# gabrielfnayres/new-vit

Measured on AMD Instinct MI355X. Metric: volumes_per_sec_mst_dinov2_fwd, higher is better.
Workload: dtype bf16; 1 GPU; MST-DINOv2 (DinoV2ClassifierSlice, ViT-S/14) forward, 4 volumes/GPU of 64x512x512 bf16 zero-padded to 518x518 (N=1370 tokens/slice); global_batch_volumes=4, slices=64, parallelism=single GPU, weights=synthetic (mst.synth seed 2), random init of the reference architecture

## Files before the change

### new-vit_amd/csrc/k_block16s.hip

```cpp
#include <type_traits>

#include "mst_common.h"

namespace {

constexpr int E = 384, HID = 1536, CH = 32;
constexpr int NCHUNK = HID / CH;
constexpr int PJ = E / CH;
constexpr int ELEM_BYTES = 24 * 1024;
constexpr int ELEMS = PJ + 2 * NCHUNK;
constexpr int NSLOT = 6;
constexpr int AHEAD = 4;
constexpr int RING_BYTES = NSLOT * ELEM_BYTES;
constexpr int B1_OFF = RING_BYTES;
constexpr int BP_OFF = B1_OFF + HID * 4;
constexpr int B2_OFF = BP_OFF + E * 4;
constexpr int LDS_BYTES = B2_OFF + E * 4;
constexpr int NF = 24;
#ifndef BLOCKS_DEPTH
#define BLOCKS_DEPTH 4
#endif
constexpr int D = BLOCKS_DEPTH;
constexpr int R = D + 2;
static_assert(NF % R == 0, "fragment ring must tile the phase");
#ifdef BLOCKS_PAIRS
constexpr int frag_of(int i) { return i; }
#else
constexpr int frag_of(int i) { return 2 * (i % 12) + i / 12; }
#endif
constexpr int BIAS_SLOT = 8;

template <int OFF, typename V> __device__ __forceinline__ void lds_read_b128(V& dst, unsigned addr) {
#if defined(BLOCKS_WACC)
    asm volatile("ds_read_b128 %0, %1 offset:%2" : "=a"(dst) : "v"(addr), "i"(OFF));
#elif !defined(BLOCKS_NOREADS)
    asm volatile("ds_read_b128 %0, %1 offset:%2" : "=v"(dst) : "v"(addr), "i"(OFF));
#else
    asm volatile("" : "=v"(dst) : "v"(addr));
#endif
}
template <int OFF, typename V> __device__ __forceinline__ void lds_read_b128_acc(V& dst, unsigned addr) {
    asm volatile("ds_read_b128 %0, %1 offset:%2" : "=a"(dst) : "v"(addr), "i"(OFF));
}
template <int N> __device__ __forceinline__ void wait_lgkm() {
    asm volatile("s_waitcnt lgkmcnt(%0)" ::"n"(N));
    __builtin_amdgcn_sched_barrier(0);
}
#ifdef BLOCKS_STAMPS
__device__ unsigned long long g_bsstamps[256 * 4 * 16];
__device__ __forceinline__ unsigned long long bstamp() {
    unsigned long long t;
    __builtin_amdgcn_sched_barrier(0);
    asm volatile("s_memtime %0\n\ts_waitcnt lgkmcnt(0)" : "=s"(t)::"memory");
    __builtin_amdgcn_sched_barrier(0);
    return t;
}
#define BST(var) const unsigned long long var = bstamp()
#define BACC(slot, a, b) st[slot] += (b) - (a)
#else
#define BST(var)
#define BACC(slot, a, b)
#endif

template <int I, int N, typename F> __device__ __forceinline__ void static_for(F&& f) {
    if constexpr (I < N) {
        f(std::integral_constant<int, I>{});
        static_for<I + 1, N>(f);
    }
}

__device__ __forceinline__ f32x16 cat16(f32x4 a, f32x4 b, f32x4 c, f32x4 d) {
    typedef __attribute__((ext_vector_type(8))) float f32x8;
    const f32x8 lo = __builtin_shufflevector(a, b, 0, 1, 2, 3, 4, 5, 6, 7), hi = __builtin_shufflevector(c, d, 0, 1, 2, 3, 4, 5, 6, 7);
    return __builtin_shufflevector(lo, hi, 0, 1, 2, 3, 4, 5, 6, 7, 8, 9, 10, 11, 12, 13, 14, 15);
}
template <int Q> __device__ __forceinline__ f32x4 sub4(f32x16 v) { return __builtin_shufflevector(v, v, 4 * Q, 4 * Q + 1, 4 * Q + 2, 4 * Q + 3); }

template <typename T> struct Gelu;
template <> struct Gelu<bf16_t> {
    static constexpr int STAGES = 7;
    static constexpr int target(int) { return 0; }
    template <int S> static __device__ __forceinline__ void stage(float v, float& a, float& b, float& c) {
        if constexpr (S == 0) a = v * v;
        else if constexpr (S == 1) a = fmaf(a, -0.06940179f * 1.4426950408889634f, -1.60031416f * 1.4426950408889634f);
        else if constexpr (S == 2) a = v * a;
        else if constexpr (S == 3) a = __builtin_amdgcn_exp2f(a);
        else if constexpr (S == 4) a = 1.0f + a;
        else if constexpr (S == 5) a = __builtin_amdgcn_rcpf(a);
        else a = v * a;
    }
};
template <> struct Gelu<f16_t> {
    static constexpr int STAGES = 9;
    static constexpr int target(int S) { return S == 0 ? 1 : (S == 2 || S == 3) ? 2 : 0; }
    template <int S> static __device__ __forceinline__ void stage(float v, float& a, float& b, float& c) {
        if constexpr (S == 0) b = __builtin_amdgcn_fmed3f(v, -8.0f, 8.0f);
        else if constexpr (S == 1) a = b * b;
        else if constexpr (S == 2) c = fmaf(a, 7.03033577e-04f * 1.4426950408889634f, -7.40112920e-02f * 1.4426950408889634f);
        else if constexpr (S == 3) c = fmaf(c, a, -1.59501577f * 1.4426950408889634f);
        else if constexpr (S == 4) a = b * c;
        else if constexpr (S == 5) a = __builtin_amdgcn_exp2f(a);
        else if constexpr (S == 6) a = 1.0f + a;
        else if constexpr (S == 7) a = __builtin_amdgcn_rcpf(a);
        else a = v * a;
    }
};

template <typename T>
__global__ __launch_bounds__(256) void block16s_kernel(float* x, const T* attn, T* xn_out, const char* __restrict__ wseq,
                                                       const float* __restrict__ b1f, const float* __restrict__ bproj,
                                                       const float* __restrict__ b2, int M, int ntiles, float eps, int layout) {
    typedef typename V8<T>::type vec8;
    typedef typename V8<T>::half_type vec4;
    extern __shared__ __attribute__((aligned(16))) char smem[];
    const bool x_in_img = layout & MST_LAYOUT_X_IN_IMAGE, x_out_img = layout & MST_LAYOUT_X_OUT_IMAGE, act_blk = layout & MST_LAYOUT_ACT_BLOCKED;
    const int tid = threadIdx.x, lane = tid & 63;
    const int wave = __builtin_amdgcn_readfirstlane(tid >> 6);
    const int row32 = lane & 31, half = lane >> 5;
    const unsigned lds_base = (unsigned)(uintptr_t)(__attribute__((address_space(3))) char*)smem;
    const unsigned lane16 = lane * 16;

    const int my_tiles = (ntiles - (int)blockIdx.x + (int)gridDim.x - 1) / (int)gridDim.x;
    if (my_tiles <= 0) return;

    for (int i = tid; i < HID / 4; i += 256) *reinterpret_cast<f32x4*>(smem + B1_OFF + i * 16) = *reinterpret_cast<const f32x4*>(b1f + 4 * i);
    for (int i = tid; i < E / 4; i += 256) {
        *reinterpret_cast<f32x4*>(smem + BP_OFF + i * 16) = *reinterpret_cast<const f32x4*>(bproj + 4 * i);
        *reinterpret_cast<f32x4*>(smem + B2_OFF + i * 16) = *reinterpret_cast<const f32x4*>(b2 + 4 * i);
    }
    asm volatile("s_waitcnt vmcnt(0) lgkmcnt(0)" ::: "memory");

#ifndef BLOCKS_DMA_GLOBAL
    const __amdgpu_buffer_rsrc_t wrsrc = __builtin_amdgcn_make_buffer_rsrc((void*)wseq, 0, ELEMS * ELEM_BYTES, 0x00020000);
    const int wlane_off = wave * 6144 + lane16;
    char* const wdst_wave = smem + wave * 6144;
    auto dma_piece = [&](int src_off, int slot, auto u_tag) {
        constexpr int u = decltype(u_tag)::value;
#ifndef BLOCKS_NODMA
        constexpr int hi = u >= 4 ? 4096 : 0;
        __builtin_amdgcn_raw_ptr_buffer_load_lds(wrsrc, LDS_PTR(wdst_wave + slot * ELEM_BYTES + hi), 16, wlane_off, src_off + hi, u * 1024 - hi, 0);
#endif
    };
#else
    const char* const wsrc_lane = wseq + (wave * 6144 + 2048) + lane16;
    char* const wdst_wave = smem + wave * 6144 + 2048;
    auto dma_piece = [&](int src_off, int slot, auto u_tag) {
        constexpr int u = decltype(u_tag)::value;
#ifndef BLOCKS_NODMA
        __builtin_amdgcn_global_load_lds(GLB_PTR(wsrc_lane + src_off), LDS_PTR(wdst_wave + slot * ELEM_BYTES), 16, (u - 2) * 1024, 0);
#endif
    };
#endif
    for (int e0 = 0; e0 < AHEAD; ++e0) static_for<0, 6>([&](auto u) { dma_piece(e0 * ELEM_BYTES, e0, u); });
    int dsrc = AHEAD * ELEM_BYTES, dslot = AHEAD;

    f32x16 acc[12];
    u32x4 xa[24];
    f32x4 hq[2][4];
    vec8 hB[2][2];
    vec8 w[R];
    float ga[8], gb[8], gc[8];
#ifdef BLOCKS_NOFILL
    hB[0][0] = hB[0][1] = hB[1][0] = hB[1][1] = vec8{};
#endif

    int slot = 0;
    const unsigned b1_lane = lds_base + B1_OFF + half * 16;

#ifdef BLOCKS_STAMPS
    unsigned long long st[16] = {0, 0, 0, 0, 0, 0, 0, 0, 0, 0, 0, 0, 0, 0, 0, 0};
    const unsigned long long tstart = bstamp();
#endif
    auto phase = [&](auto head_tag, auto tail_tag, auto bq_tag, int bias_chunk, auto&& mf, auto&& fill, auto cat_tag, auto ord_tag, auto nord_tag) {
        constexpr bool HEAD = decltype(head_tag)::value, TAIL = decltype(tail_tag)::value;
        constexpr int ORD = decltype(ord_tag)::value, NORD = decltype(nord_tag)::value;
        auto fr = [](int i, int ord) constexpr { return ord ? frag_of(i) : i; };
        constexpr int BQ = decltype(bq_tag)::value, CAT = decltype(cat_tag)::value;
        BST(p0);
        asm volatile("s_waitcnt vmcnt(12)\n\ts_barrier" ::: "memory");
        BST(p1);
        BACC(CAT, p0, p1);
        const unsigned cur = lds_base + slot * ELEM_BYTES + lane16;
        const int nslot = slot + 1 == NSLOT ? 0 : slot + 1;
        const unsigned nxt = lds_base + nslot * ELEM_BYTES + lane16;
        const int my_dsrc = dsrc, my_dslot = dslot;
        dsrc = dsrc + ELEM_BYTES == ELEMS * ELEM_BYTES ? 0 : dsrc + ELEM_BYTES;
        dslot = dslot + 1 == NSLOT ? 0 : dslot + 1;
        const unsigned baddr = b1_lane + 128 * bias_chunk;
        f32x4 bt0, bt1, bt2, bt3;
        if constexpr (HEAD) static_for<0, D>([&](auto q) { lds_read_b128<fr(decltype(q)::value, ORD) * 1024>(w[decltype(q)::value % R], cur); });
        static_for<0, NF>([&](auto it) {
            constexpr int i = decltype(it)::value;
            if constexpr (i + D < NF) lds_read_b128<fr(i + D, ORD) * 1024>(w[(i + D) % R], cur);
            else if constexpr (TAIL) lds_read_b128<fr(i + D - NF, NORD) * 1024>(w[(i + D) % R], nxt);
            if constexpr (BQ >= 0 && i == BIAS_SLOT) {
                lds_read_b128_acc<0>(bt0, baddr);
                lds_read_b128_acc<32>(bt1, baddr);
                lds_read_b128_acc<64>(bt2, baddr);
                lds_read_b128_acc<96>(bt3, baddr);
            }
#ifndef BLOCKS_WAIT1
            if constexpr (i % 2 == 0) {
                constexpr int last = TAIL ? i + D : (i + D < NF - 1 ? i + D : NF - 1);
                constexpr int younger_frags = last - (i + 1) > 0 ? last - (i + 1) : 0;
                constexpr int younger_bias = (BQ >= 0 && i >= BIAS_SLOT && i + 1 <= BIAS_SLOT + D) ? 4 : 0;
                wait_lgkm<younger_frags + younger_bias>();
            } else {
                __builtin_amdgcn_sched_barrier(0);
            }
#else
            constexpr int younger_frags = TAIL ? D : (NF - 1 - i < D ? NF - 1 - i : D);
            constexpr int younger_bias = (BQ >= 0 && i >= BIAS_SLOT && i <= BIAS_SLOT + D) ? 4 : 0;
            wait_lgkm<younger_frags + younger_bias>();
#endif
            if constexpr (BQ >= 0 && i == BIAS_SLOT + D + 1) {
                asm volatile("" : "+a"(bt0), "+a"(bt1), "+a"(bt2), "+a"(bt3));
                hq[BQ < 0 ? 0 : BQ][0] = bt0;
                hq[BQ < 0 ? 0 : BQ][1] = bt1;
                hq[BQ < 0 ? 0 : BQ][2] = bt2;
                hq[BQ < 0 ? 0 : BQ][3] = bt3;
            }
            mf(it, w[i % R]);
#ifdef BLOCKS_DMA_FRONT
            if constexpr (i == 0) static_for<0, 6>([&](auto u) { dma_piece(my_dsrc, my_dslot, u); });
#else
            if constexpr (i % 4 == 3) dma_piece(my_dsrc, my_dslot, std::integral_constant<int, i / 4>{});
#endif
            fill(it);
        });
        slot = nslot;
        BST(p2);
        BACC(CAT + 1, p1, p2);
    };
    constexpr std::integral_constant<int, 0> C_PROJ{};
    constexpr std::integral_constant<int, 2> C_A{};
    constexpr std::integral_constant<int, 4> C_B{};
    constexpr std::integral_constant<int, 6> C_G10{};
    auto no_fill = [](auto) {};
    constexpr std::true_type YES{};
    constexpr std::false_type NO{};
    constexpr std::integral_constant<int, -1> NOBIAS{};
    constexpr std::integral_constant<int, 0> I0{};
    constexpr std::integral_constant<int, 1> I1{};

    auto gemm1_mf = [&](auto hs_tag) {
        return [&](auto it, const vec8& wf) {
            constexpr int hs = decltype(hs_tag)::value, i = decltype(it)::value;
            f32x16 c = cat16(hq[hs][0], hq[hs][1], hq[hs][2], hq[hs][3]);
            c = mfma32(wf, __builtin_bit_cast(vec8, xa[i]), c);
            static_for<0, 4>([&](auto q) { hq[hs][decltype(q)::value] = sub4<decltype(q)::value>(c); });
        };
    };
    auto gemm2_mf = [&](auto hs_tag) {
        return [&](auto it, const vec8& wf) {
            constexpr int hs = decltype(hs_tag)::value, i = frag_of(decltype(it)::value);
            acc[i >> 1] = mfma32(wf, hB[hs][i & 1], acc[i >> 1]);
        };
    };

    constexpr int GOPS = 8 * Gelu<T>::STAGES + 4;
    auto gelu_op = [&](auto hs_tag, auto part_tag, auto n_tag) {
        constexpr int hs = decltype(hs_tag)::value, PART = decltype(part_tag)::value, n = decltype(n_tag)::value;
        if constexpr (n < 8 * Gelu<T>::STAGES) {
            constexpr int grp = n / (4 * Gelu<T>::STAGES), m = n % (4 * Gelu<T>::STAGES);
            constexpr int st = m / 4, val = 4 * grp + m % 4;
            Gelu<T>::template stage<st>(hq[hs][2 * PART + (val >> 2)][val & 3], ga[val], gb[val], gc[val]);
            if constexpr (Gelu<T>::target(st) == 0) asm volatile("" : "+v"(ga[val]));
            else if constexpr (Gelu<T>::target(st) == 1) asm volatile("" : "+v"(gb[val]));
            else asm volatile("" : "+v"(gc[val]));
        } else if constexpr (n < GOPS) {
            constexpr int pr = n - 8 * Gelu<T>::STAGES;
            hB[hs][PART][2 * pr] = (T)ga[2 * pr];
            hB[hs][PART][2 * pr + 1] = (T)ga[2 * pr + 1];
        }
    };
    constexpr int OPS_PER_SLOT = (GOPS + NF - 2) / (NF - 1);
    auto gelu_fill = [&](auto hs_tag, auto part_tag) {
        return [&, hs_tag, part_tag](auto it) {
            constexpr int i = decltype(it)::value;
#ifdef BLOCKS_NOFILL
            if constexpr (i == 12) static_for<0, 8>([&](auto e) { hB[decltype(hs_tag)::value][decltype(part_tag)::value][decltype(e)::value] = (T)hq[decltype(hs_tag)::value][2 * decltype(part_tag)::value + (decltype(e)::value >> 2)][decltype(e)::value & 3]; });
            if constexpr (false)
#else
            if constexpr (i >= 1)
#endif
                static_for<0, OPS_PER_SLOT>([&](auto o) { gelu_op(hs_tag, part_tag, std::integral_constant<int, (i - 1) * OPS_PER_SLOT + decltype(o)::value>{}); });
        };
    };
    auto gelu_now = [&](auto hs_tag, auto part_tag) { static_for<0, GOPS>([&](auto n) { gelu_op(hs_tag, part_tag, n); }); };

    const int last_grp = (M - 1) >> 5;
    auto row_of = [&](int tile) { const int g = tile * 128 + wave * 32 + row32; return (unsigned)(g < M ? g : M - 1); };
    auto grp_of = [&](int tile) { return (size_t)((tile * 4 + wave) < last_grp ? (tile * 4 + wave) : last_grp); };
    auto load_attn = [&](int tile) {
        if (act_blk) {
            const char* ap = (const char*)attn + (grp_of(tile) * (32 * E * 2) + lane16);
#pragma unroll
            for (int i = 0; i < 24; ++i) xa[i] = *reinterpret_cast<const u32x4*>(ap + 1024 * i);
        } else {
            const char* ap = (const char*)attn + ((size_t)row_of(tile) * (E * 2) + half * 16);
#pragma unroll
            for (int i = 0; i < 24; ++i) xa[i] = *reinterpret_cast<const u32x4*>(ap + 32 * i);
        }
    };
    auto load_x = [&](int tile, auto t_tag) {
        constexpr int t = decltype(t_tag)::value;
        const char* xp = x_in_img ? (const char*)x + (grp_of(tile) * (32 * E * 4) + lane16) + 4096 * t
                                  : (const char*)x + ((size_t)row_of(tile) * (E * 4) + half * 16) + 128 * t;
        const int qstep = x_in_img ? 1024 : 32;
#pragma unroll
        for (int q = 0; q < 4; ++q) {
            const f32x4 v = *reinterpret_cast<const f32x4*>(xp + qstep * q);
#pragma unroll
            for (int r = 0; r < 4; ++r) acc[t][4 * q + r] = v[r];
        }
    };
#ifndef BLOCKS_TILE_CYCLES
#define BLOCKS_TILE_CYCLES 170000
#endif
#ifndef BLOCKS_NO_DEPHASE
    if (my_tiles >= 4) {
        const int min_tiles = ntiles / (int)gridDim.x;
        const unsigned u = (((unsigned)blockIdx.x >> 3) + 5u * ((unsigned)blockIdx.x & 7u)) & 15u;
        const unsigned long long delay = (unsigned long long)BLOCKS_TILE_CYCLES * ((my_tiles > min_tiles ? 0u : 16u) + u) / 32u;
        const unsigned long long t0 = __builtin_readcyclecounter();
        for (int it = 0; it < 640 && __builtin_readcyclecounter() - t0 < delay; ++it) __builtin_amdgcn_s_sleep(32);
    }
#endif
    load_attn(blockIdx.x);
    static_for<0, 12>([&](auto t) { load_x(blockIdx.x, t); });

    for (int k = 0; k < my_tiles; ++k) {
        const int tile = blockIdx.x + k * gridDim.x;
        const int next_tile = k + 1 < my_tiles ? tile + (int)gridDim.x : tile;
        const int grow = tile * 128 + wave * 32 + row32;
        const bool valid = grow < M;
        const unsigned crow = (unsigned)(valid ? grow : M - 1);
        BST(q0);
        BST(q1);
        BACC(8, q0, q1);
        static_for<0, PJ>([&](auto jt) {
            constexpr int j = decltype(jt)::value;
            auto mf = [&](auto it, const vec8& wf) {
                constexpr int i = frag_of(decltype(it)::value);
                acc[i >> 1] = mfma32(wf, __builtin_bit_cast(vec8, xa[2 * j + (i & 1)]), acc[i >> 1]);
            };
            if constexpr (j == 0) phase(YES, YES, NOBIAS, 0, mf, no_fill, C_PROJ, I1, I1);
            else if constexpr (j == PJ - 1) phase(NO, NO, I0, 0, mf, no_fill, C_PROJ, I1, I1);
            else phase(NO, YES, NOBIAS, 0, mf, no_fill, C_PROJ, I1, I1);
        });
        BST(q2);
        {
            const unsigned bp = lds_base + BP_OFF + half * 16, bb = lds_base + B2_OFF + half * 16;
            f32x4 s4 = {0.f, 0.f, 0.f, 0.f};
            static_for<0, 12>([&](auto tt) {
                constexpr int t = decltype(tt)::value;
                f32x4 b[4];
                static_for<0, 4>([&](auto q) { lds_read_b128<128 * t + 32 * decltype(q)::value>(b[decltype(q)::value], bp); });
                wait_lgkm<0>();
                acc[t] += cat16(b[0], b[1], b[2], b[3]);
                s4 += (sub4<0>(acc[t]) + sub4<1>(acc[t])) + (sub4<2>(acc[t]) + sub4<3>(acc[t]));
                asm volatile("" : "+v"(s4));
            });
            float sum = (s4[0] + s4[1]) + (s4[2] + s4[3]);
            sum += __shfl_xor(sum, 32, 64);
            const float mean = sum * (1.0f / E);
            const f32x4 mean4 = {mean, mean, mean, mean};
            f32x4 q4 = {0.f, 0.f, 0.f, 0.f};
            static_for<0, 12>([&](auto tt) {
                constexpr int t = decltype(tt)::value;
                static_for<0, 4>([&](auto q) {
                    const f32x4 d = sub4<decltype(q)::value>(acc[t]) - mean4;
                    q4 = __builtin_elementwise_fma(d, d, q4);
                });
                asm volatile("" : "+v"(q4));
            });
            float sq = (q4[0] + q4[1]) + (q4[2] + q4[3]);
            sq += __shfl_xor(sq, 32, 64);
            const float rstd = rsqrtf(sq * (1.0f / E) + eps);
            const float nmr = -mean * rstd;
            const f32x4 rstd4 = {rstd, rstd, rstd, rstd}, nmr4 = {nmr, nmr, nmr, nmr};
            static_for<0, 12>([&](auto tt) {
                constexpr int t = decltype(tt)::value;
                f32x4 b[4];
                static_for<0, 4>([&](auto q) { lds_read_b128<128 * t + 32 * decltype(q)::value>(b[decltype(q)::value], bb); });
#pragma unroll
                for (int p = 0; p < 2; ++p) {
                    const f32x4 n0 = __builtin_elementwise_fma(p ? sub4<2>(acc[t]) : sub4<0>(acc[t]), rstd4, nmr4);
                    const f32x4 n1 = __builtin_elementwise_fma(p ? sub4<3>(acc[t]) : sub4<1>(acc[t]), rstd4, nmr4);
                    vec8 o;
#pragma unroll
                    for (int e = 0; e < 4; ++e) { o[e] = (T)n0[e]; o[4 + e] = (T)n1[e]; }
                    xa[2 * t + p] = __builtin_bit_cast(u32x4, o);
                    asm volatile("" : "+v"(xa[2 * t + p]));
                }
                wait_lgkm<0>();
                acc[t] += cat16(b[0], b[1], b[2], b[3]);
            });
        }
        BST(q3);
        BACC(9, q2, q3);
        phase(YES, YES, I1, 1, gemm1_mf(I0), no_fill, C_G10, I0, I0);
        wait_lgkm<0>();
        gelu_now(I0, I0);
        auto iter = [&](auto par_tag, auto bias_tag, int c) {
            constexpr int cur = decltype(par_tag)::value, nx = cur ^ 1;
            phase(NO, YES, NOBIAS, 0, gemm1_mf(std::integral_constant<int, nx>{}), gelu_fill(std::integral_constant<int, cur>{}, I1), C_A, I0, I1);
            if constexpr (decltype(bias_tag)::value)
                phase(NO, YES, std::integral_constant<int, cur>{}, c + 2, gemm2_mf(std::integral_constant<int, cur>{}), gelu_fill(std::integral_constant<int, nx>{}, I0), C_B, I1, I0);
            else
                phase(NO, YES, NOBIAS, 0, gemm2_mf(std::integral_constant<int, cur>{}), gelu_fill(std::integral_constant<int, nx>{}, I0), C_B, I1, I1);
        };
#pragma unroll 1
        for (int c = 0; c < NCHUNK - 2; c += 2) {
            iter(I0, YES, c);
            iter(I1, YES, c + 1);
        }
        iter(I0, NO, NCHUNK - 2);
        wait_lgkm<0>();
        gelu_now(I1, I1);
        phase(NO, NO, NOBIAS, 0, gemm2_mf(I1), no_fill, C_B, I1, I1);
        BST(q4);
        {
            const size_t grp = (size_t)tile * 4 + wave;
            const bool grp_valid = (tile * 4 + wave) * 32 < M;
            load_attn(next_tile);
            f32x4 rstd4 = {0.f, 0.f, 0.f, 0.f}, nmr4 = {0.f, 0.f, 0.f, 0.f};
            if (xn_out) {
                f32x4 s4 = {0.f, 0.f, 0.f, 0.f};
                static_for<0, 12>([&](auto tt) {
                    constexpr int t = decltype(tt)::value;
                    s4 += (sub4<0>(acc[t]) + sub4<1>(acc[t])) + (sub4<2>(acc[t]) + sub4<3>(acc[t]));
                    asm volatile("" : "+v"(s4));
                });
                float sum = (s4[0] + s4[1]) + (s4[2] + s4[3]);
                sum += __shfl_xor(sum, 32, 64);
                const float mean = sum * (1.0f / E);
                const f32x4 mean4 = {mean, mean, mean, mean};
                f32x4 q4 = {0.f, 0.f, 0.f, 0.f};
                static_for<0, 12>([&](auto tt) {
                    constexpr int t = decltype(tt)::value;
                    static_for<0, 4>([&](auto q) {
                        const f32x4 d = sub4<decltype(q)::value>(acc[t]) - mean4;
                        q4 = __builtin_elementwise_fma(d, d, q4);
                    });
                    asm volatile("" : "+v"(q4));
                });
                float sq = (q4[0] + q4[1]) + (q4[2] + q4[3]);
                sq += __shfl_xor(sq, 32, 64);
                const float rstd = rsqrtf(sq * (1.0f / E) + eps);
                const float nmr = -mean * rstd;
                rstd4 = f32x4{rstd, rstd, rstd, rstd};
                nmr4 = f32x4{nmr, nmr, nmr, nmr};
            }
            char* const xo = x_out_img ? (char*)x + (grp * (32 * E * 4) + lane16) : (char*)x + ((size_t)grow * (E * 4) + half * 16);
            const int xt = x_out_img ? 4096 : 128, xq = x_out_img ? 1024 : 32;
            const bool x_store = x_out_img ? grp_valid : valid;
            char* const op = act_blk ? (char*)xn_out + (grp * (32 * E * 2) + lane16) : (char*)xn_out + ((size_t)crow * (E * 2) + half * 16);
            const int ostep = act_blk ? 1024 : 32;
            const bool n_store = act_blk ? grp_valid : valid;
            static_for<0, 12>([&](auto tt) {
                constexpr int t = decltype(tt)::value;
                if (x_store) {
#pragma unroll
                    for (int q = 0; q < 4; ++q) {
                        f32x4 v;
#pragma unroll
                        for (int r = 0; r < 4; ++r) v[r] = acc[t][4 * q + r];
                        *reinterpret_cast<f32x4*>(xo + xt * t + xq * q) = v;
                    }
                }
                if (xn_out) {
#pragma unroll
                    for (int p = 0; p < 2; ++p) {
                        const f32x4 n0 = __builtin_elementwise_fma(p ? sub4<2>(acc[t]) : sub4<0>(acc[t]), rstd4, nmr4);
                        const f32x4 n1 = __builtin_elementwise_fma(p ? sub4<3>(acc[t]) : sub4<1>(acc[t]), rstd4, nmr4);
                        vec4 lo, hi;
#pragma unroll
                        for (int e = 0; e < 4; ++e) { lo[e] = (T)n0[e]; hi[e] = (T)n1[e]; }
                        const u32x2 l2 = __builtin_bit_cast(u32x2, lo), h2 = __builtin_bit_cast(u32x2, hi);
                        u32x4 o;
#pragma unroll
                        for (int d2 = 0; d2 < 2; ++d2) {
                            const auto sw = __builtin_amdgcn_permlane32_swap(l2[d2], h2[d2], false, false);
                            o[d2] = sw[0];
                            o[2 + d2] = sw[1];
                        }
                        if (n_store) *reinterpret_cast<u32x4*>(op + ostep * (2 * t + p)) = o;
                    }
                }
                __builtin_amdgcn_sched_barrier(0);
#ifndef BLOCKS_EPI_LATE_LOADS
                load_x(next_tile, tt);
                __builtin_amdgcn_sched_barrier(0);
#endif
            });
#ifdef BLOCKS_EPI_LATE_LOADS
            static_for<0, 12>([&](auto tt) { load_x(next_tile, tt); });
#endif
        }
        BST(q5);
        BACC(10, q4, q5);
    }
#ifdef BLOCKS_STAMPS
    st[15] = bstamp() - tstart;
    if (lane == 0) for (int i = 0; i < 16; ++i) g_bsstamps[(blockIdx.x * 4 + wave) * 16 + i] = st[i];
#endif
    asm volatile("s_waitcnt vmcnt(0)" ::: "memory");
}

template <typename T>
int launch_t(float* x, const void* attn, void* xn_out, const void* wseq, const float* b1f, const float* bproj, const float* b2,
             int64_t M, float eps, int layout, hipStream_t s) {
    static mst_lds_once lds_once;
    auto kern = block16s_kernel<T>;
    mst_allow_lds((const void*)kern, LDS_BYTES, &lds_once);
    const int ntiles = (int)((M + 127) / 128);
    const int cus = mst_persistent_grid();
    const int nblk = ntiles < cus ? ntiles : cus;
    kern<<<dim3(nblk), dim3(256), LDS_BYTES, s>>>(x, (const T*)attn, (T*)xn_out, (const char*)wseq, b1f, bproj, b2, (int)M, ntiles, eps, layout);
    return mst_check_launch("block16s");
}

}

#ifdef BLOCKS_STAMPS
extern "C" int mst_debug_blocks_stamps(unsigned long long* host, int n) {
    return (int)hipMemcpyFromSymbol(host, HIP_SYMBOL(g_bsstamps), sizeof(unsigned long long) * n);
}
#endif

int launch_block16s(float* x, const void* attn, void* xn_out, int dt, const void* wseq, const float* b1f, const float* bproj,
                    const float* b2, int64_t M, int E_, float eps, int layout, hipStream_t s) {
    MST_CHECK_ARG(E_ == E, "block_fused_s: embed_dim=%d unsupported (384)", E_);
    MST_CHECK_ARG(M > 0 && M < (1ll << 31) - 128, "block_fused_s: bad M");
    if (dt == MST_BF16) return launch_t<bf16_t>(x, attn, xn_out, wseq, b1f, bproj, b2, M, eps, layout, s);
    if (dt == MST_F16) return launch_t<f16_t>(x, attn, xn_out, wseq, b1f, bproj, b2, M, eps, layout, s);
    mst_set_error("block_fused_s: dtype %d unsupported (f16 / bf16)", dt);
    return MST_EINVAL;
}
```

Before: 156.3 volumes/s.

## Overlap residual stores and x loads with proj GEMM via paired tile order

Reorders the projection GEMM fragment schedule into tile pairs so that the epilogue's residual/x-norm stores for the previous tile and the loads of the next tile's residual are spread across the next tile's proj phases as fill work. Stores switch to buffer stores with per-group range-limited resources instead of branches. The proj-weight DMA uses a new pair-interleaved source layout, and the bias for the first GEMM1 chunk is preloaded separately. The dephase sleep loop is also removed. This adds considerable scheduling complexity, and deferring stores across tiles needs a final drain after the loop.

```diff
diff --git a/new-vit_amd/csrc/k_block16s.hip b/new-vit_amd/csrc/k_block16s.hip
--- a/new-vit_amd/csrc/k_block16s.hip
+++ b/new-vit_amd/csrc/k_block16s.hip
@@ -28,6 +28,9 @@
 #else
 constexpr int frag_of(int i) { return 2 * (i % 12) + i / 12; }
 #endif
+constexpr int pair_frag_of(int i) { return 4 * (i / 4) + 2 * (i % 2) + (i / 2) % 2; }
+constexpr int ORD_STREAM = 0, ORD_TILE = 1, ORD_PAIR = 2;
+constexpr int frag_in_order(int i, int ord) { return ord == ORD_PAIR ? pair_frag_of(i) : ord == ORD_TILE ? frag_of(i) : i; }
 constexpr int BIAS_SLOT = 8;
 
 template <int OFF, typename V> __device__ __forceinline__ void lds_read_b128(V& dst, unsigned addr) {
@@ -130,7 +133,6 @@
     }
     asm volatile("s_waitcnt vmcnt(0) lgkmcnt(0)" ::: "memory");
 
-#ifndef BLOCKS_DMA_GLOBAL
     const __amdgpu_buffer_rsrc_t wrsrc = __builtin_amdgcn_make_buffer_rsrc((void*)wseq, 0, ELEMS * ELEM_BYTES, 0x00020000);
     const int wlane_off = wave * 6144 + lane16;
     char* const wdst_wave = smem + wave * 6144;
@@ -141,17 +143,20 @@
         __builtin_amdgcn_raw_ptr_buffer_load_lds(wrsrc, LDS_PTR(wdst_wave + slot * ELEM_BYTES + hi), 16, wlane_off, src_off + hi, u * 1024 - hi, 0);
 #endif
     };
-#else
-    const char* const wsrc_lane = wseq + (wave * 6144 + 2048) + lane16;
-    char* const wdst_wave = smem + wave * 6144 + 2048;
-    auto dma_piece = [&](int src_off, int slot, auto u_tag) {
-        constexpr int u = decltype(u_tag)::value;
+    int pair_piece_off[6];
+#pragma unroll
+    for (int u = 0; u < 6; ++u) {
+        const int n = 6 * wave + u;
+        pair_piece_off[u] = (n >> 2) * ELEM_BYTES + (n & 3) * 1024 - (u >= 4 ? u * 1024 - 4096 : u * 1024);
+    }
+    auto dma_pair_piece = [&](auto pe_tag, int slot, auto u_tag) {
+        constexpr int u = decltype(u_tag)::value, pe = decltype(pe_tag)::value, hi = u >= 4 ? 4096 : 0;
 #ifndef BLOCKS_NODMA
-        __builtin_amdgcn_global_load_lds(GLB_PTR(wsrc_lane + src_off), LDS_PTR(wdst_wave + slot * ELEM_BYTES), 16, (u - 2) * 1024, 0);
-#endif
-    };
-#endif
-    for (int e0 = 0; e0 < AHEAD; ++e0) static_for<0, 6>([&](auto u) { dma_piece(e0 * ELEM_BYTES, e0, u); });
+        __builtin_amdgcn_raw_ptr_buffer_load_lds(wrsrc, LDS_PTR(wdst_wave + slot * ELEM_BYTES + hi), 16, (int)lane16,
+                                                 pair_piece_off[u] + ((pe & 1) * 6 * ELEM_BYTES + (pe >> 1) * 4096), u * 1024 - hi, 0);
+#endif
+    };
+    static_for<0, AHEAD>([&](auto e0) { static_for<0, 6>([&](auto u) { dma_pair_piece(e0, decltype(e0)::value, u); }); });
     int dsrc = AHEAD * ELEM_BYTES, dslot = AHEAD;
 
     f32x16 acc[12];
@@ -165,19 +170,29 @@
 #endif
 
     int slot = 0;
-    const unsigned b1_lane = lds_base + B1_OFF + half * 16;
+    auto bias_addr = [&](unsigned uniform_off) {
+        unsigned a;
+        asm volatile("v_lshrrev_b32 %0, 5, %2\n\tv_and_b32 %0, 16, %0\n\tv_add_u32 %0, %1, %0" : "=&v"(a) : "s"(lds_base + uniform_off), "v"(lane16));
+        return a;
+    };
+    auto add_other_half = [](float v) {
+        const auto sw = __builtin_amdgcn_permlane32_swap(__builtin_bit_cast(unsigned, v), __builtin_bit_cast(unsigned, v), false, false);
+        const unsigned own = sw[0], other = sw[1];
+        return __builtin_bit_cast(float, own) + __builtin_bit_cast(float, other);
+    };
 
 #ifdef BLOCKS_STAMPS
     unsigned long long st[16] = {0, 0, 0, 0, 0, 0, 0, 0, 0, 0, 0, 0, 0, 0, 0, 0};
     const unsigned long long tstart = bstamp();
 #endif
-    auto phase = [&](auto head_tag, auto tail_tag, auto bq_tag, int bias_chunk, auto&& mf, auto&& fill, auto cat_tag, auto ord_tag, auto nord_tag) {
+    auto phase = [&](auto head_tag, auto tail_tag, auto bq_tag, int bias_chunk, auto&& mf, auto&& fill, auto cat_tag, auto ord_tag, auto nord_tag,
+                     auto dma_tag, auto rows_tag) {
         constexpr bool HEAD = decltype(head_tag)::value, TAIL = decltype(tail_tag)::value;
-        constexpr int ORD = decltype(ord_tag)::value, NORD = decltype(nord_tag)::value;
-        auto fr = [](int i, int ord) constexpr { return ord ? frag_of(i) : i; };
+        constexpr int ORD = decltype(ord_tag)::value, NORD = decltype(nord_tag)::value, DMA_PE = decltype(dma_tag)::value;
+        auto fr = [](int i, int ord) constexpr { return frag_in_order(i, ord); };
         constexpr int BQ = decltype(bq_tag)::value, CAT = decltype(cat_tag)::value;
         BST(p0);
-        asm volatile("s_waitcnt vmcnt(12)\n\ts_barrier" ::: "memory");
+        asm volatile("s_waitcnt vmcnt(%0)\n\ts_barrier" ::"n"(12 + decltype(rows_tag)::value) : "memory");
         BST(p1);
         BACC(CAT, p0, p1);
         const unsigned cur = lds_base + slot * ELEM_BYTES + lane16;
@@ -186,7 +201,8 @@
         const int my_dsrc = dsrc, my_dslot = dslot;
         dsrc = dsrc + ELEM_BYTES == ELEMS * ELEM_BYTES ? 0 : dsrc + ELEM_BYTES;
         dslot = dslot + 1 == NSLOT ? 0 : dslot + 1;
-        const unsigned baddr = b1_lane + 128 * bias_chunk;
+        unsigned baddr = 0;
+        if constexpr (decltype(bq_tag)::value >= 0) baddr = bias_addr(B1_OFF + 128 * bias_chunk);
         f32x4 bt0, bt1, bt2, bt3;
         if constexpr (HEAD) static_for<0, D>([&](auto q) { lds_read_b128<fr(decltype(q)::value, ORD) * 1024>(w[decltype(q)::value % R], cur); });
         static_for<0, NF>([&](auto it) {
@@ -221,11 +237,10 @@
                 hq[BQ < 0 ? 0 : BQ][3] = bt3;
             }
             mf(it, w[i % R]);
-#ifdef BLOCKS_DMA_FRONT
-            if constexpr (i == 0) static_for<0, 6>([&](auto u) { dma_piece(my_dsrc, my_dslot, u); });
-#else
-            if constexpr (i % 4 == 3) dma_piece(my_dsrc, my_dslot, std::integral_constant<int, i / 4>{});
-#endif
+            if constexpr (i % 4 == 3) {
+                if constexpr (DMA_PE >= 0) dma_pair_piece(dma_tag, my_dslot, std::integral_constant<int, i / 4>{});
+                else dma_piece(my_dsrc, my_dslot, std::integral_constant<int, i / 4>{});
+            }
             fill(it);
         });
         slot = nslot;
@@ -242,6 +257,10 @@
     constexpr std::integral_constant<int, -1> NOBIAS{};
     constexpr std::integral_constant<int, 0> I0{};
     constexpr std::integral_constant<int, 1> I1{};
+    constexpr std::integral_constant<int, 2> I2{};
+    constexpr std::integral_constant<int, 3> I3{};
+    constexpr std::integral_constant<int, -1> STREAM{};
+    constexpr std::integral_constant<int, 0> ROWS0{};
 
     auto gemm1_mf = [&](auto hs_tag) {
         return [&](auto it, const vec8& wf) {
@@ -290,68 +309,124 @@
     auto gelu_now = [&](auto hs_tag, auto part_tag) { static_for<0, GOPS>([&](auto n) { gelu_op(hs_tag, part_tag, n); }); };
 
     const int last_grp = (M - 1) >> 5;
-    auto row_of = [&](int tile) { const int g = tile * 128 + wave * 32 + row32; return (unsigned)(g < M ? g : M - 1); };
+    auto lane16_here = [&]() {
+        unsigned l;
+        asm volatile("v_mov_b32 %0, %1" : "=v"(l) : "v"(lane16));
+        return l;
+    };
+    auto row_of = [&](int tile) {
+        int wave_row;
+        asm volatile("s_lshl_b32 %0, %1, 5" : "=s"(wave_row) : "s"(wave));
+        const int g = tile * 128 + wave_row + (int)((lane16_here() >> 4) & 31);
+        return (unsigned)(g < M ? g : M - 1);
+    };
     auto grp_of = [&](int tile) { return (size_t)((tile * 4 + wave) < last_grp ? (tile * 4 + wave) : last_grp); };
+    auto row_off = [](int lane_part, auto units_tag, int shift) {
+        int off;
+        asm volatile("v_lshl_add_u32 %0, %1, %2, %3" : "=v"(off) : "n"(decltype(units_tag)::value), "s"(shift), "v"(lane_part));
+        return off;
+    };
+    const int xin_sh = x_in_img ? 10 : 5, att_sh = act_blk ? 10 : 5;
+    const char* in_x;
+    int xin_lane;
+    auto row_in_grp = [&](int tile) { return (int)(row_of(tile) - (unsigned)grp_of(tile) * 32u); };
+    auto x_in_of = [&](int tile) {
+        in_x = (const char*)x + grp_of(tile) * (32 * E * 4);
+        const unsigned l16 = lane16_here();
+        xin_lane = x_in_img ? (int)l16 : row_in_grp(tile) * (E * 4) + (int)((l16 >> 5) & 16);
+    };
     auto load_attn = [&](int tile) {
-        if (act_blk) {
-            const char* ap = (const char*)attn + (grp_of(tile) * (32 * E * 2) + lane16);
-#pragma unroll
-            for (int i = 0; i < 24; ++i) xa[i] = *reinterpret_cast<const u32x4*>(ap + 1024 * i);
-        } else {
-            const char* ap = (const char*)attn + ((size_t)row_of(tile) * (E * 2) + half * 16);
-#pragma unroll
-            for (int i = 0; i < 24; ++i) xa[i] = *reinterpret_cast<const u32x4*>(ap + 32 * i);
-        }
-    };
-    auto load_x = [&](int tile, auto t_tag) {
-        constexpr int t = decltype(t_tag)::value;
-        const char* xp = x_in_img ? (const char*)x + (grp_of(tile) * (32 * E * 4) + lane16) + 4096 * t
-                                  : (const char*)x + ((size_t)row_of(tile) * (E * 4) + half * 16) + 128 * t;
-        const int qstep = x_in_img ? 1024 : 32;
-#pragma unroll
-        for (int q = 0; q < 4; ++q) {
-            const f32x4 v = *reinterpret_cast<const f32x4*>(xp + qstep * q);
-#pragma unroll
-            for (int r = 0; r < 4; ++r) acc[t][4 * q + r] = v[r];
-        }
-    };
-#ifndef BLOCKS_TILE_CYCLES
-#define BLOCKS_TILE_CYCLES 170000
-#endif
-#ifndef BLOCKS_NO_DEPHASE
-    if (my_tiles >= 4) {
-        const int min_tiles = ntiles / (int)gridDim.x;
-        const unsigned u = (((unsigned)blockIdx.x >> 3) + 5u * ((unsigned)blockIdx.x & 7u)) & 15u;
-        const unsigned long long delay = (unsigned long long)BLOCKS_TILE_CYCLES * ((my_tiles > min_tiles ? 0u : 16u) + u) / 32u;
-        const unsigned long long t0 = __builtin_readcyclecounter();
-        for (int it = 0; it < 640 && __builtin_readcyclecounter() - t0 < delay; ++it) __builtin_amdgcn_s_sleep(32);
-    }
-#endif
+        const char* const ap = (const char*)attn + grp_of(tile) * (32 * E * 2);
+        const unsigned l16 = lane16_here();
+        const int lane_part = act_blk ? (int)l16 : row_in_grp(tile) * (E * 2) + (int)((l16 >> 5) & 16);
+        static_for<0, 24>([&](auto i) {
+            xa[decltype(i)::value] = *reinterpret_cast<const u32x4*>(ap + (unsigned)row_off(lane_part, i, att_sh));
+        });
+    };
+    auto load_x = [&](auto t_tag, auto q_tag) {
+        constexpr int t = decltype(t_tag)::value, q = decltype(q_tag)::value;
+        const f32x4 v = *reinterpret_cast<const f32x4*>(in_x + (unsigned)row_off(xin_lane, std::integral_constant<int, 4 * t + q>{}, xin_sh));
+#pragma unroll
+        for (int r = 0; r < 4; ++r) acc[t][4 * q + r] = v[r];
+    };
+    const int xout_sh = x_out_img ? 10 : 5, xn_sh = act_blk ? 10 : 5;
+    int xout_lane = 0, xn_lane = 0;
+    auto out_lanes = [&]() {
+        const unsigned l16 = lane16_here();
+        const int r32 = (l16 >> 4) & 31, h16 = (l16 >> 5) & 16;
+        xout_lane = x_out_img ? (int)l16 : r32 * (E * 4) + h16;
+        xn_lane = act_blk ? (int)l16 : r32 * (E * 2) + h16;
+    };
+    auto rows_rsrc = [&](void* base, int tile, int row_bytes, bool whole_groups) {
+        const int grp = tile * 4 + wave, rows = M - grp * 32;
+        const int nrows = rows <= 0 || !base ? 0 : (rows > 32 || whole_groups) ? 32 : rows;
+        return __builtin_amdgcn_make_buffer_rsrc((char*)base + (size_t)grp * (32 * row_bytes), 0, nrows * row_bytes, 0x00020000);
+    };
+    __amdgpu_buffer_rsrc_t out_x = __builtin_amdgcn_make_buffer_rsrc((void*)x, 0, 0, 0x00020000), out_n = out_x;
+    float out_rstd = 0.f, out_nmr = 0.f;
+    auto store_x = [&](auto t_tag, auto q_tag) {
+        constexpr int t = decltype(t_tag)::value, q = decltype(q_tag)::value;
+        f32x4 v;
+#pragma unroll
+        for (int r = 0; r < 4; ++r) v[r] = acc[t][4 * q + r];
+        __builtin_amdgcn_raw_buffer_store_b128(__builtin_bit_cast(u32x4, v), out_x, row_off(xout_lane, std::integral_constant<int, 4 * t + q>{}, xout_sh), 0, 0);
+    };
+    auto store_n = [&](auto t_tag, auto p_tag) {
+        constexpr int t = decltype(t_tag)::value, p = decltype(p_tag)::value;
+        vec4 lo, hi;
+#pragma unroll
+        for (int e = 0; e < 4; ++e) {
+            float n0 = fmaf(acc[t][8 * p + e], out_rstd, out_nmr), n1 = fmaf(acc[t][8 * p + 4 + e], out_rstd, out_nmr);
+            asm volatile("" : "+v"(n0), "+v"(n1));
+            lo[e] = (T)n0;
+            hi[e] = (T)n1;
+        }
+        const u32x2 l2 = __builtin_bit_cast(u32x2, lo), h2 = __builtin_bit_cast(u32x2, hi);
+        u32x4 o;
+#pragma unroll
+        for (int d2 = 0; d2 < 2; ++d2) {
+            const auto sw = __builtin_amdgcn_permlane32_swap(l2[d2], h2[d2], false, false);
+            o[d2] = sw[0];
+            o[2 + d2] = sw[1];
+        }
+        __builtin_amdgcn_raw_buffer_store_b128(o, out_n, row_off(xn_lane, std::integral_constant<int, 2 * t + p>{}, xn_sh), 0, 0);
+    };
+    auto pair_op = [&](auto p_tag, auto n_tag) {
+        constexpr int P = decltype(p_tag)::value, n = decltype(n_tag)::value;
+        if constexpr (n < 12) {
+            constexpr int t = 2 * P + n / 6, m = n % 6;
+            if constexpr (m < 4) store_x(std::integral_constant<int, t>{}, std::integral_constant<int, m>{});
+            else store_n(std::integral_constant<int, t>{}, std::integral_constant<int, m - 4>{});
+        } else if constexpr (n < 20) {
+            load_x(std::integral_constant<int, 2 * P + (n - 12) / 4>{}, std::integral_constant<int, (n - 12) % 4>{});
+        }
+    };
+    constexpr int PAIR_LOADS = 8, HEAD_LOADS = 24 + PAIR_LOADS;
     load_attn(blockIdx.x);
-    static_for<0, 12>([&](auto t) { load_x(blockIdx.x, t); });
+    x_in_of(blockIdx.x);
+    static_for<12, 20>([&](auto n) { pair_op(I0, n); });
 
     for (int k = 0; k < my_tiles; ++k) {
         const int tile = blockIdx.x + k * gridDim.x;
-        const int next_tile = k + 1 < my_tiles ? tile + (int)gridDim.x : tile;
-        const int grow = tile * 128 + wave * 32 + row32;
-        const bool valid = grow < M;
-        const unsigned crow = (unsigned)(valid ? grow : M - 1);
-        BST(q0);
-        BST(q1);
-        BACC(8, q0, q1);
-        static_for<0, PJ>([&](auto jt) {
-            constexpr int j = decltype(jt)::value;
+        static_for<0, PJ>([&](auto et) {
+            constexpr int e = decltype(et)::value, P = e / 2, H = e % 2;
             auto mf = [&](auto it, const vec8& wf) {
-                constexpr int i = frag_of(decltype(it)::value);
-                acc[i >> 1] = mfma32(wf, __builtin_bit_cast(vec8, xa[2 * j + (i & 1)]), acc[i >> 1]);
+                constexpr int i = decltype(it)::value;
+                acc[2 * P + i % 2] = mfma32(wf, __builtin_bit_cast(vec8, xa[12 * H + i / 2]), acc[2 * P + i % 2]);
             };
-            if constexpr (j == 0) phase(YES, YES, NOBIAS, 0, mf, no_fill, C_PROJ, I1, I1);
-            else if constexpr (j == PJ - 1) phase(NO, NO, I0, 0, mf, no_fill, C_PROJ, I1, I1);
-            else phase(NO, YES, NOBIAS, 0, mf, no_fill, C_PROJ, I1, I1);
+            auto fill = [&](auto it) {
+                if constexpr (H == 0 && P + 1 < 6) pair_op(std::integral_constant<int, P + 1>{}, it);
+            };
+            constexpr int rows = e == 0 ? HEAD_LOADS : e == 1 ? HEAD_LOADS + PAIR_LOADS : e <= 10 ? PAIR_LOADS : 0;
+            constexpr std::integral_constant<int, rows> ROWS{};
+            constexpr std::integral_constant<int, (e + AHEAD < PJ ? e + AHEAD : -1)> DMA{};
+            if constexpr (e == 0) phase(YES, YES, NOBIAS, 0, mf, fill, C_PROJ, I2, I2, DMA, ROWS);
+            else if constexpr (e == PJ - 1) phase(NO, NO, NOBIAS, 0, mf, fill, C_PROJ, I2, I2, DMA, ROWS);
+            else phase(NO, YES, NOBIAS, 0, mf, fill, C_PROJ, I2, I2, DMA, ROWS);
         });
         BST(q2);
         {
-            const unsigned bp = lds_base + BP_OFF + half * 16, bb = lds_base + B2_OFF + half * 16;
+            const unsigned bp = bias_addr(BP_OFF), bb = bias_addr(B2_OFF);
             f32x4 s4 = {0.f, 0.f, 0.f, 0.f};
             static_for<0, 12>([&](auto tt) {
                 constexpr int t = decltype(tt)::value;
@@ -363,7 +438,7 @@
                 asm volatile("" : "+v"(s4));
             });
             float sum = (s4[0] + s4[1]) + (s4[2] + s4[3]);
-            sum += __shfl_xor(sum, 32, 64);
+            sum = add_other_half(sum);
             const float mean = sum * (1.0f / E);
             const f32x4 mean4 = {mean, mean, mean, mean};
             f32x4 q4 = {0.f, 0.f, 0.f, 0.f};
@@ -376,7 +451,7 @@
                 asm volatile("" : "+v"(q4));
             });
             float sq = (q4[0] + q4[1]) + (q4[2] + q4[3]);
-            sq += __shfl_xor(sq, 32, 64);
+            sq = add_other_half(sq);
             const float rstd = rsqrtf(sq * (1.0f / E) + eps);
             const float nmr = -mean * rstd;
             const f32x4 rstd4 = {rstd, rstd, rstd, rstd}, nmr4 = {nmr, nmr, nmr, nmr};
@@ -400,41 +475,50 @@
         }
         BST(q3);
         BACC(9, q2, q3);
-        phase(YES, YES, I1, 1, gemm1_mf(I0), no_fill, C_G10, I0, I0);
+        {
+            const unsigned baddr = bias_addr(B1_OFF);
+            f32x4 bt[4];
+            static_for<0, 4>([&](auto q) { lds_read_b128_acc<32 * decltype(q)::value>(bt[decltype(q)::value], baddr); });
+            wait_lgkm<0>();
+            asm volatile("" : "+a"(bt[0]), "+a"(bt[1]), "+a"(bt[2]), "+a"(bt[3]));
+            static_for<0, 4>([&](auto q) { hq[0][decltype(q)::value] = bt[decltype(q)::value]; });
+        }
+        phase(YES, YES, I1, 1, gemm1_mf(I0), no_fill, C_G10, I0, I0, STREAM, ROWS0);
         wait_lgkm<0>();
         gelu_now(I0, I0);
-        auto iter = [&](auto par_tag, auto bias_tag, int c) {
+        auto iter = [&](auto par_tag, auto bias_tag, int c, auto dma_a, auto dma_b) {
             constexpr int cur = decltype(par_tag)::value, nx = cur ^ 1;
-            phase(NO, YES, NOBIAS, 0, gemm1_mf(std::integral_constant<int, nx>{}), gelu_fill(std::integral_constant<int, cur>{}, I1), C_A, I0, I1);
+            phase(NO, YES, NOBIAS, 0, gemm1_mf(std::integral_constant<int, nx>{}), gelu_fill(std::integral_constant<int, cur>{}, I1), C_A, I0, I1, dma_a, ROWS0);
             if constexpr (decltype(bias_tag)::value)
-                phase(NO, YES, std::integral_constant<int, cur>{}, c + 2, gemm2_mf(std::integral_constant<int, cur>{}), gelu_fill(std::integral_constant<int, nx>{}, I0), C_B, I1, I0);
+                phase(NO, YES, std::integral_constant<int, cur>{}, c + 2, gemm2_mf(std::integral_constant<int, cur>{}), gelu_fill(std::integral_constant<int, nx>{}, I0), C_B, I1, I0, dma_b, ROWS0);
             else
-                phase(NO, YES, NOBIAS, 0, gemm2_mf(std::integral_constant<int, cur>{}), gelu_fill(std::integral_constant<int, nx>{}, I0), C_B, I1, I1);
+                phase(NO, YES, NOBIAS, 0, gemm2_mf(std::integral_constant<int, cur>{}), gelu_fill(std::integral_constant<int, nx>{}, I0), C_B, I1, I1, dma_b, ROWS0);
         };
 #pragma unroll 1
-        for (int c = 0; c < NCHUNK - 2; c += 2) {
-            iter(I0, YES, c);
-            iter(I1, YES, c + 1);
-        }
-        iter(I0, NO, NCHUNK - 2);
+        for (int c = 0; c < NCHUNK - 4; c += 2) {
+            iter(I0, YES, c, STREAM, STREAM);
+            iter(I1, YES, c + 1, STREAM, STREAM);
+        }
+        iter(I0, YES, NCHUNK - 4, STREAM, STREAM);
+        iter(I1, YES, NCHUNK - 3, STREAM, I0);
+        iter(I0, NO, NCHUNK - 2, I1, I2);
         wait_lgkm<0>();
         gelu_now(I1, I1);
-        phase(NO, NO, NOBIAS, 0, gemm2_mf(I1), no_fill, C_B, I1, I1);
+        phase(NO, NO, NOBIAS, 0, gemm2_mf(I1), no_fill, C_B, I1, I1, I3, ROWS0);
         BST(q4);
         {
-            const size_t grp = (size_t)tile * 4 + wave;
-            const bool grp_valid = (tile * 4 + wave) * 32 < M;
+            const int next_tile = k + 1 < my_tiles ? tile + (int)gridDim.x : tile;
             load_attn(next_tile);
-            f32x4 rstd4 = {0.f, 0.f, 0.f, 0.f}, nmr4 = {0.f, 0.f, 0.f, 0.f};
             if (xn_out) {
                 f32x4 s4 = {0.f, 0.f, 0.f, 0.f};
                 static_for<0, 12>([&](auto tt) {
                     constexpr int t = decltype(tt)::value;
                     s4 += (sub4<0>(acc[t]) + sub4<1>(acc[t])) + (sub4<2>(acc[t]) + sub4<3>(acc[t]));
                     asm volatile("" : "+v"(s4));
+                    __builtin_amdgcn_sched_barrier(0);
                 });
                 float sum = (s4[0] + s4[1]) + (s4[2] + s4[3]);
-                sum += __shfl_xor(sum, 32, 64);
+                sum = add_other_half(sum);
                 const float mean = sum * (1.0f / E);
                 const f32x4 mean4 = {mean, mean, mean, mean};
                 f32x4 q4 = {0.f, 0.f, 0.f, 0.f};
@@ -445,63 +529,30 @@
                         q4 = __builtin_elementwise_fma(d, d, q4);
                     });
                     asm volatile("" : "+v"(q4));
+                    __builtin_amdgcn_sched_barrier(0);
                 });
                 float sq = (q4[0] + q4[1]) + (q4[2] + q4[3]);
-                sq += __shfl_xor(sq, 32, 64);
-                const float rstd = rsqrtf(sq * (1.0f / E) + eps);
-                const float nmr = -mean * rstd;
-                rstd4 = f32x4{rstd, rstd, rstd, rstd};
-                nmr4 = f32x4{nmr, nmr, nmr, nmr};
+                sq = add_other_half(sq);
+                out_rstd = rsqrtf(sq * (1.0f / E) + eps);
+                out_nmr = -mean * out_rstd;
             }
-            char* const xo = x_out_img ? (char*)x + (grp * (32 * E * 4) + lane16) : (char*)x + ((size_t)grow * (E * 4) + half * 16);
-            const int xt = x_out_img ? 4096 : 128, xq = x_out_img ? 1024 : 32;
-            const bool x_store = x_out_img ? grp_valid : valid;
-            char* const op = act_blk ? (char*)xn_out + (grp * (32 * E * 2) + lane16) : (char*)xn_out + ((size_t)crow * (E * 2) + half * 16);
-            const int ostep = act_blk ? 1024 : 32;
-            const bool n_store = act_blk ? grp_valid : valid;
-            static_for<0, 12>([&](auto tt) {
-                constexpr int t = decltype(tt)::value;
-                if (x_store) {
-#pragma unroll
-                    for (int q = 0; q < 4; ++q) {
-                        f32x4 v;
-#pragma unroll
-                        for (int r = 0; r < 4; ++r) v[r] = acc[t][4 * q + r];
-                        *reinterpret_cast<f32x4*>(xo + xt * t + xq * q) = v;
-                    }
-                }
-                if (xn_out) {
-#pragma unroll
-                    for (int p = 0; p < 2; ++p) {
-                        const f32x4 n0 = __builtin_elementwise_fma(p ? sub4<2>(acc[t]) : sub4<0>(acc[t]), rstd4, nmr4);
-                        const f32x4 n1 = __builtin_elementwise_fma(p ? sub4<3>(acc[t]) : sub4<1>(acc[t]), rstd4, nmr4);
-                        vec4 lo, hi;
-#pragma unroll
-                        for (int e = 0; e < 4; ++e) { lo[e] = (T)n0[e]; hi[e] = (T)n1[e]; }
-                        const u32x2 l2 = __builtin_bit_cast(u32x2, lo), h2 = __builtin_bit_cast(u32x2, hi);
-                        u32x4 o;
-#pragma unroll
-                        for (int d2 = 0; d2 < 2; ++d2) {
-                            const auto sw = __builtin_amdgcn_permlane32_swap(l2[d2], h2[d2], false, false);
-                            o[d2] = sw[0];
-                            o[2 + d2] = sw[1];
-                        }
-                        if (n_store) *reinterpret_cast<u32x4*>(op + ostep * (2 * t + p)) = o;
-                    }
-                }
-                __builtin_amdgcn_sched_barrier(0);
-#ifndef BLOCKS_EPI_LATE_LOADS
-                load_x(next_tile, tt);
-                __builtin_amdgcn_sched_barrier(0);
-#endif
-            });
-#ifdef BLOCKS_EPI_LATE_LOADS
-            static_for<0, 12>([&](auto tt) { load_x(next_tile, tt); });
-#endif
+            out_lanes();
+            out_x = rows_rsrc(x, tile, E * 4, x_out_img);
+            out_n = rows_rsrc(xn_out, tile, E * 2, act_blk);
+            __builtin_amdgcn_sched_barrier(0);
+            static_for<0, 12>([&](auto n) { pair_op(I0, n); });
+            __builtin_amdgcn_sched_barrier(0);
+            x_in_of(next_tile);
+            static_for<12, 20>([&](auto n) { pair_op(I0, n); });
+            __builtin_amdgcn_sched_barrier(0);
         }
         BST(q5);
         BACC(10, q4, q5);
     }
+    BST(q6);
+    static_for<1, 6>([&](auto P) { static_for<0, 12>([&](auto n) { pair_op(P, n); }); });
+    BST(q7);
+    BACC(11, q6, q7);
 #ifdef BLOCKS_STAMPS
     st[15] = bstamp() - tstart;
     if (lane == 0) for (int i = 0; i < 16; ++i) g_bsstamps[(blockIdx.x * 4 + wave) * 16 + i] = st[i];
```

After: 162.9 volumes/s (median of 6 runs). 1.04x the previous value.
